# AlexTate/ShortSeq

Measured on AMD Instinct MI355X. Metric: nt/sec 2-bit encode (32/96/512-nt batches) + hamming pairs/sec; % HBM roofline, higher is better.
Workload: dtype u8; 1 GPU; C2: 100M x 32-nt batch encode (short_seq_64 path) per GPU; reads_per_gpu=100000000, read_len=32, global_batch=100000000, parallelism=dp1 (read shards, no collective)

## Files before the change

### shortseq_amd/csrc/ss_counter.hip

```cpp
#include "ss_device.h"
#include "ss_internal.h"

using namespace ssd;

namespace {
struct alignas(16) Slot {
    unsigned long long key;
    uint32_t ncount;
    uint32_t first;
};
static_assert(sizeof(Slot) == 16, "one slot = one dwordx4");
constexpr uint32_t kNoFirst = 0xFFFFFFFFu;
constexpr uint64_t kMaxIndex = 0xFFFFFFFEull;
constexpr unsigned long long kOvfTable = 1ull, kOvfExtract = 2ull, kOvfField = 4ull, kOvfIndex = 8ull;
constexpr int kThreads = 256;
constexpr uint32_t kMaxParts = 64;
constexpr uint32_t kExtractBlocks = 4096;
constexpr uint32_t kExtractT = 64;
constexpr uint32_t kSliceLogMax = 11;
constexpr uint32_t kMwSliceLog = 11;
constexpr uint32_t kPartBlocks = 1024;
constexpr uint32_t kMaxRegions = 32768;
}

// ... 1156 lines not shown
        const bool heavy_tile = any_heavy != 0;
#pragma unroll
        for (int j = 0; j < (int)(kTile / T); ++j) {
            const uint32_t e = j * T + threadIdx.x;
            if (e < cnt) {
                const uint32_t sp = lstart[lb[j]] + rank[j];
                skey[sp] = key[j];
                sidx[sp] = idx[j];
            }
        }
        if (heavy_tile)
            for (uint32_t i = threadIdx.x; i < kTile; i += T) ht[i] = 0;
        __syncthreads();
        if (heavy_tile) {
            for (uint32_t i0 = 0; i0 < cnt; i0 += T) {
                const uint32_t i = i0 + threadIdx.x;
                const uint64_t k = i < cnt ? skey[i] : 0ull;
                const uint32_t x = i < cnt ? sidx[i] : kWeighted;
                const bool act = i < cnt && lcount[region_of_h(t, k) - r0] > heavy_at && !(x & kWeighted);
                if (!act) continue;
                uint32_t h = dedup_home(k, kHtLog);
                for (;;) {
                    uint32_t e = ht[h];
                    if (e == 0) {
                        e = atomicCAS(&ht[h], 0u, (i + 1) | (1u << 16));
                        if (e == 0) break;
                    }
                    const uint32_t j = (e & 0xFFFFu) - 1;
                    if (skey[j] == k) {
                        atomicAdd(&ht[h], 1u << 16);
                        atomicMin(&sidx[j], x);
                        sidx[i] = kDead;
                        break;
                    }
                    h = (h + 1) & (kTile - 1);
                }
            }
            __syncthreads();
            for (uint32_t i = threadIdx.x; i < cnt; i += T) {
                const uint32_t b = region_of_h(t, skey[i]) - r0;
                if (lcount[b] > heavy_at && sidx[i] != kDead) atomicAdd(&hcnt[b], 1u);
            }
            for (uint32_t i = threadIdx.x; i < nb; i += T)
                if (lcount[i] > heavy_at) lstart[i] = 0;
            __syncthreads();
        }
#pragma unroll
        for (int j = 0; j < (int)(kTile / T); ++j) asm volatile("" ::"v"(nkey[j]), "v"(nidx[j]));
        for (uint32_t i = threadIdx.x; i < cnt; i += T) {
            const uint64_t k = skey[i];
            const uint32_t x = sidx[i];
            if (x == kDead) continue;
            const uint32_t b = region_of_h(t, k) - r0;
            uint32_t local, c = 1;
            if (heavy_tile && lcount[b] > heavy_at) {
                local = atomicAdd(&lstart[b], 1u);
                if (!(x & kWeighted)) {
                    uint32_t h = dedup_home(k, kHtLog);
                    while ((ht[h] & 0xFFFFu) != i + 1) h = (h + 1) & (kTile - 1);
                    c = ht[h] >> 16;
                }
            } else {
                local = i - lstart[b];
            }
            uint32_t xi = x;
            if (x & kWeighted) {
                const uint32_t p = x & ~kWeighted;
                xi = srec[p].idx;
                c = src_cnt[p];
            } else if (c > 1) {
                xi = x | kWeighted;
            }
            const uint32_t gpos = cursor[b] + local;
            if (w.slab && gpos >= sbase + (b + 1) * ssize) {
                const uint64_t sp = atomicAdd(w.spill_ctr, 1u);
                const uint64_t key = k * kSlotInv;
                if (sp < w.spill_cap)
                    w.spill[sp] = make_uint4((uint32_t)key, (uint32_t)(key >> 32), c, xi & ~kWeighted);
                else
                    atomicOr(t.overflow, kOvfTable);
                continue;
            }
            if (c > 1) w.bcnt[gpos] = c;
            Rec12 r;
            r.klo = (uint32_t)k;
            r.khi = (uint32_t)(k >> 32);
            r.idx = xi;
            ((Rec12*)w.keys)[gpos] = r;
        }
        __syncthreads();
        for (uint32_t i = threadIdx.x; i < nb; i += T)
            cursor[i] += (heavy_tile && lcount[i] > heavy_at) ? hcnt[i] : lcount[i];
        __syncthreads();
    }
    for (uint32_t i = threadIdx.x; i < nb; i += T)
        w.seg_end[(uint64_t)fb * nb + i] = w.slab ? min(cursor[i], sbase + (i + 1) * ssize) : cursor[i];
}

__global__ __launch_bounds__(256) void k_spill_insert(Tbl t, PartWs w, const uint32_t* __restrict__ fill,
                                                      uint64_t base_index) {
    const uint64_t m = min((uint64_t)fill[fill_at(kSpillCtr)], w.spill_cap);
    for (uint64_t i0 = (uint64_t)blockIdx.x * 256; i0 < m; i0 += (uint64_t)gridDim.x * 256) {
        const uint64_t i = i0 + threadIdx.x;
        const uint4 r = w.spill[min(i, m - 1)];
        const uint64_t k = ((uint64_t)r.y << 32) | r.x;
        bool act = i < m;
        uint32_t c = r.z, idx = r.w;
        wave_fold<kSpillFold, true>(act, k, c, idx);
        if (act && tbl_add(t, k, c, base_index + idx) && t.occ && k != kEmpty) atomicAdd(&t.occ[region_of(t, k)], 1u);
    }
}


constexpr uint32_t kAggSliceT = 512;
constexpr int kAggP = 4;


constexpr int kAggProbe = 2;
constexpr int kAggProbeS = 4;
template <int G>
__device__ __forceinline__ bool lds_probe_round(unsigned long long* skey, uint32_t mask, uint64_t empty, uint64_t k,
                                                uint32_t& off, uint32_t& done, uint32_t& at) {
    const uint32_t S = mask + 1;
    unsigned long long cur[G];
#pragma unroll
    for (int g = 0; g < G; ++g) cur[g] = skey[(off + g) & mask];
    int hit = -1;
    bool free_at = false;
#pragma unroll
    for (int g = G - 1; g >= 0; --g) {
        if (cur[g] == k) {
            hit = g;
            free_at = false;
        } else if (cur[g] == empty) {
            hit = g;
            free_at = true;
        }
    }
    if (hit >= 0) {
        at = (off + (uint32_t)hit) & mask;
        if (!free_at) return true;
        const unsigned long long prev = atomicCAS(&skey[at], (unsigned long long)empty, (unsigned long long)k);
        if (prev == empty || prev == k) return true;
        off = (at + 1) & mask;
        done += (uint32_t)hit + 1;
    } else {
        off = (off + G) & mask;
        done += G;
    }
    at = S;
    return done >= S;
}

template <int T, bool REC12>
__global__ __launch_bounds__(T) void k_pc_aggregate_slice(Tbl t, PartWs w, uint64_t base_index, bool fresh = false) {
    const uint32_t S = (uint32_t)t.slice_mask + 1;
    extern __shared__ __attribute__((aligned(16))) unsigned char smem[];
    unsigned long long* skey = (unsigned long long*)smem;
    uint32_t* bcnt = (uint32_t*)(skey + S);
    uint32_t* bfst = bcnt + S;
    __shared__ uint32_t sent[3];
    const uint32_t region = blockIdx.x;
    const uint64_t slice_base = (uint64_t)region << t.slice_log;
    static_assert(kFinePerBin <= 32, "segment table: two lanes per segment");
    const uint32_t lane = threadIdx.x & 63u;
    uint32_t meta;
    if (w.seg_end) {
        const uint32_t rpb = 1u << (w.rbits - kCoarseBits);
        const uint32_t sg = lane % kFinePerBin;
        const uint64_t at = (uint64_t)((region / rpb) * kFinePerBin + sg) * rpb + region % rpb;
        meta = (lane < kFinePerBin ? w.hist : w.seg_end)[at];
    } else {
        meta = w.rstart[region + (lane & 1u)];
    }
    constexpr uint64_t kE = REC12 ? kEmptyH : kEmpty;
    if (fresh) {
        for (uint32_t i = threadIdx.x; i < S; i += T) skey[i] = kE;
    } else {
        for (uint32_t i = threadIdx.x; i < S; i += T) {
            const uint64_t k = t.slots[slice_base + i].key;
            skey[i] = REC12 ? (k == kEmpty ? kEmptyH : k * kSlotMul) : k;
        }
    }
    for (uint32_t i = threadIdx.x; i < S; i += T) {
        bcnt[i] = 0;
        bfst[i] = 0xFFFFFFFFu;
    }
    if (threadIdx.x == 0) {
        sent[0] = 0;
        sent[1] = 0xFFFFFFFFu;
        sent[2] = 0;
    }
    constexpr int kP = kAggP;
    uint32_t seg0[kFinePerBin], pre[kFinePerBin + 1];
    pre[0] = 0;
    if (w.seg_end) {
#pragma unroll
        for (uint32_t sg = 0; sg < kFinePerBin; ++sg) {
            seg0[sg] = (uint32_t)__builtin_amdgcn_readlane((int)meta, (int)sg);
            pre[sg + 1] = pre[sg] + ((uint32_t)__builtin_amdgcn_readlane((int)meta, (int)(kFinePerBin + sg)) - seg0[sg]);
        }
    } else {
        seg0[0] = (uint32_t)__builtin_amdgcn_readlane((int)meta, 0);
        const uint32_t end = (uint32_t)__builtin_amdgcn_readlane((int)meta, 1);
#pragma unroll
        for (uint32_t sg = 0; sg < kFinePerBin; ++sg) pre[sg + 1] = end - seg0[0];
    }
    const uint32_t total = pre[kFinePerBin];
    auto flat_at = [&](uint32_t f) -> uint32_t {
        uint32_t e = seg0[0] + f;
#pragma unroll
        for (uint32_t sg = 1; sg < kFinePerBin; ++sg)
            if (f >= pre[sg]) e = seg0[sg] + (f - pre[sg]);
        return e;
    };
    uint64_t nkey[kP];
    uint32_t nidx[kP], nel[kP];
    auto load_step = [&](uint32_t e0) {
#pragma unroll
        for (int q = 0; q < kP; ++q) {
            const uint32_t f = min(e0 + q * T + threadIdx.x, total - 1u);
            nel[q] = flat_at(f);
            if constexpr (REC12) {
                const Rec12 r = w.brec[nel[q]];
                nkey[q] = ((uint64_t)r.khi << 32) | r.klo;
                nidx[q] = r.idx;
            } else {
                nkey[q] = w.bkey[nel[q]];
                nidx[q] = w.bidx[nel[q]];
            }
        }
    };
    if (total) load_step(0);
    auto home_of = [&](uint64_t k) -> uint64_t {
        return REC12 ? (t.shift >= 64 ? 0ull : k >> t.shift) : slot_top(t, k);
    };
    auto probe_round = [&](uint64_t k, uint32_t& off, uint32_t& done, uint32_t& at) -> bool {
        return lds_probe_round<kAggProbe>(skey, (uint32_t)t.slice_mask, kE, k, off, done, at);
    };
    auto probe_round_s = [&](uint64_t k, uint32_t& off, uint32_t& done, uint32_t& at) -> bool {
        return lds_probe_round<kAggProbeS>(skey, (uint32_t)t.slice_mask, kE, k, off, done, at);
    };
    auto commit = [&](uint32_t at, uint32_t c, uint32_t ix) {
        if (at == S) {
            atomicOr(t.overflow, kOvfTable);
        } else {
            atomicAdd(&bcnt[at], c);
            atomicMin(&bfst[at], ix);
        }
    };
    __syncthreads();
    for (uint32_t e0 = 0; e0 < total; e0 += kP * T) {
        uint64_t key[kP];
        uint32_t idx[kP], el[kP];
#pragma unroll
        for (int q = 0; q < kP; ++q) {
            key[q] = nkey[q];
            idx[q] = nidx[q];
            el[q] = nel[q];
        }
        uint32_t cw[kP];
#pragma unroll
        for (int q = 0; q < kP; ++q) {
            const bool valid = e0 + q * T + threadIdx.x < total;
            cw[q] = (valid && (idx[q] & kWeighted)) ? w.bcnt[el[q]] : 1u;
        }
        load_step(e0 + kP * T);
        uint32_t pend = 0, soff[kP];
#pragma unroll
        for (int q = 0; q < kP; ++q) {
            const bool valid = e0 + q * T + threadIdx.x < total;
            soff[q] = 0;
            if (valid && key[q] == kE) {
                atomicAdd(&sent[0], cw[q]);
                atomicMin(&sent[1], idx[q] & ~kWeighted);
            }
            if (!valid || key[q] == kE) continue;
            uint32_t off = (uint32_t)(home_of(key[q]) & t.slice_mask), done = 0, at;
            if (probe_round(key[q], off, done, at))
                commit(at, cw[q], idx[q] & ~kWeighted);
            else {
                pend |= 1u << q;
                soff[q] = off;
            }
        }
        if (__ballot(pend != 0)) {
            uint64_t k = 0;
            uint32_t off = 0, done = 0, c = 0, ix = 0;
            auto pick = [&]() {
#pragma unroll
                for (int q = kP - 1; q >= 0; --q)
                    if (pend & (1u << q)) {
                        k = key[q];
                        off = soff[q];
                        c = cw[q];
                        ix = idx[q] & ~kWeighted;
                    }
                done = (off - (uint32_t)home_of(k)) & (uint32_t)t.slice_mask;
            };
            if (pend) pick();
            while (__ballot(pend != 0)) {
                uint32_t at;
                if (pend && probe_round_s(k, off, done, at)) {
                    commit(at, c, ix);
                    pend &= pend - 1u;
                    if (pend) pick();
                }
            }
        }
    }
    __syncthreads();
    uint32_t used = 0;
    uint4* sl = (uint4*)&t.slots[slice_base];
    for (uint32_t i = threadIdx.x; i < S; i += T) {
        const unsigned long long kh = skey[i];
        used += kh != kE ? 1u : 0u;
        const unsigned long long k = REC12 ? (kh != kE ? kh * kSlotInv : kEmpty) : kh;
        const uint32_t bc = bcnt[i];
        if (fresh) {
            sl[i] = make_uint4((uint32_t)k, (uint32_t)(k >> 32), ~bc,
                               bc ? (uint32_t)(base_index + bfst[i]) : kNoFirst);
        } else if (bc) {
            const uint4 old = sl[i];
            const uint32_t f = (uint32_t)(base_index + bfst[i]);
            sl[i] = make_uint4((uint32_t)k, (uint32_t)(k >> 32), old.z - bc, f < old.w ? f : old.w);
        }
    }
    if (t.occ) {
        if (used) atomicAdd(&sent[2], used);
        __syncthreads();
        if (threadIdx.x == 0) t.occ[region] = sent[2];
    }
    if (threadIdx.x == 0 && sent[0]) {
        Slot* ss = &t.slots[t.mask + 1];
        atomicAdd(&ss->ncount, 0u - sent[0]);
        atomicMin(&ss->first, (uint32_t)(base_index + sent[1]));
    }
}

struct TripleRecs {
    const uint64_t* keys;
    const uint64_t* counts;
    const uint64_t* first;
    __device__ __forceinline__ uint64_t key(uint64_t j) const { return keys[j]; }
    __device__ __forceinline__ void load(uint64_t j, uint32_t, uint64_t& k, unsigned long long& c,
                                         unsigned long long& f) const {
        k = keys[j];
        c = counts[j];
        f = first[j];
    }
};

struct PackedRecs {
    const uint4* rec;
    const uint64_t* run_base;
    __device__ __forceinline__ uint64_t key(uint64_t j) const {
        const uint4 v = rec[j];
        return ((uint64_t)v.y << 32) | v.x;
    }
    __device__ __forceinline__ void load(uint64_t j, uint32_t run, uint64_t& k, unsigned long long& c,
                                         unsigned long long& f) const {
        const uint4 v = rec[j];
        k = ((uint64_t)v.y << 32) | v.x;
        c = v.z;
        f = run_base[run] + v.w;
    }
};

template <typename Recs>
__device__ __forceinline__ uint32_t run_rel(const Tbl& t, const Recs& recs, uint64_t j, uint32_t reg_lo, uint32_t nreg) {
    const uint64_t k = recs.key(j);
    if (k == kEmpty) return nreg;
    const uint32_t r = region_of(t, k);
    return r < reg_lo ? 0u : min(r - reg_lo, nreg);
}

template <typename Recs>
__global__ __launch_bounds__(256) void k_run_bounds(Tbl t, Recs recs,
                                                   const uint64_t* __restrict__ run_off, uint32_t n_runs,
                                                   uint32_t reg_lo, uint32_t nreg, uint32_t* __restrict__ bounds) {
    const uint64_t i = (uint64_t)blockIdx.x * 256 + threadIdx.x;
    uint32_t run = 0;
    while (run < n_runs && !(run_off[2 * run] <= i && i < run_off[2 * run + 1])) ++run;
    if (run == n_runs) return;
    const uint64_t beg = run_off[2 * run], end = run_off[2 * run + 1];
    auto rel = [&](uint64_t j) { return run_rel(t, recs, j, reg_lo, nreg); };
    const uint32_t r = rel(i);
    const uint32_t prev = i == beg ? 0u : rel(i - 1) + 1u;
    uint32_t* b = bounds + (uint64_t)run * (nreg + 1);
    for (uint32_t q = (i == beg ? 0u : prev); q <= r; ++q) b[q] = (uint32_t)(i - beg);
    if (i + 1 == end)
        for (uint32_t q = r + 1; q <= nreg; ++q) b[q] = (uint32_t)(end - beg);
}

constexpr uint32_t kMergeT = 512;
constexpr uint32_t kMergeSearchRuns = 64;
constexpr int kMergeK = 4;

template <typename Recs>
__global__ __launch_bounds__(kMergeT) void k_merge_runs(Tbl t, Recs recs,
                                                       const uint64_t* __restrict__ run_off, uint32_t n_runs,
                                                       uint32_t reg_lo, uint32_t nreg,
                                                       const uint32_t* __restrict__ bounds) {
    extern __shared__ __attribute__((aligned(16))) unsigned char smem[];
    const uint32_t S = (uint32_t)t.slice_mask + 1;
    unsigned long long* skey = (unsigned long long*)smem;
    uint32_t* scnt = (uint32_t*)(skey + S);
    uint32_t* sfst = scnt + S;
    const uint32_t j = blockIdx.x;
    const uint64_t base = (uint64_t)(reg_lo + j) << t.slice_log;
    uint4* sl = (uint4*)&t.slots[base];
    for (uint32_t q = threadIdx.x; q < S; q += kMergeT) {
        const uint4 v = sl[q];
        skey[q] = ((uint64_t)v.y << 32) | v.x;
        scnt[q] = ~v.z;
        sfst[q] = v.w;
    }
    __shared__ uint32_t s_lo[kMergeSearchRuns], s_hi[kMergeSearchRuns];
    if (!bounds) {
        const uint32_t hl = threadIdx.x & 31u, hsh = threadIdx.x & 32u;
        for (uint32_t q = threadIdx.x >> 5; q < 2 * n_runs; q += kMergeT / 32) {
            const uint32_t run = q >> 1, target = j + (q & 1u);
            const uint64_t beg = run_off[2 * run], end = run_off[2 * run + 1];
            uint64_t L = beg, H = end;
            while (H > L) {
                const uint64_t len = H - L;
                const uint64_t p = L + len * hl / 32;
                const bool below = run_rel(t, recs, p, reg_lo, nreg) < target;
                const uint32_t c = (uint32_t)__popcll((__ballot(below) >> hsh) & 0xFFFFFFFFull);
                if (c == 0) break;
                const uint64_t nx = c < 32 ? L + len * c / 32 : H;
                L = L + len * (c - 1) / 32 + 1;
                H = nx;
            }
            if (hl == 0) ((q & 1u) ? s_hi : s_lo)[run] = (uint32_t)(L - beg);
        }
    }
// ... 1414 lines not shown
    c->ws_bidx = nullptr;
    c->ws_bcnt = nullptr;
    c->ws_spill = nullptr;
    c->ws_reads = 0;
    c->ws_slab = 0;
    c->ws_brecs = 0;
    return SS_OK;
}

static int insert_impl(ss_counter* c, const uint8_t* d_ascii, uint64_t n, uint32_t L, uint64_t stride,
                       uint64_t base_index, uint64_t* d_first_bad, void* stream, const uint64_t* words_in,
                       const uint64_t* keys_in = nullptr) {
    hipStream_t s = (hipStream_t)stream;
    int rc = SS_OK;
    if (keys_in) {
        if (c->W != 1) return ss_fail(SS_EARG, "precomputed keys need a single-word handle");
        if (n == 0) return SS_OK;
        if (n > c->ws_reads && (rc = ss_counter_reserve(c, n)) != SS_OK) return rc;
    }
    const uint32_t rb = c->log2cap - c->slice_log;
    const bool opt = !words_in && n > 0 && n <= c->ws_reads && rb > kCoarseBits && rb - kCoarseBits <= 8 &&
                     (keys_in || (d_ascii && (L == 16 || L == 32) && stride % 16 == 0 && (((uintptr_t)d_ascii) & 15) == 0));
    if (keys_in) {
    } else if (!words_in) {
        if (!d_first_bad) return ss_fail(SS_EARG, "d_first_bad is required");
        if (stride < L) return ss_fail(SS_EARG, "stride < L");
        if ((rc = fix_length(c, L))) return rc;
        if (!opt) rc = ss_check(set_u64(d_first_bad, true, s), "reset first_bad");
        if (rc || n == 0) return rc;
        if (!d_ascii) return ss_fail(SS_EARG, "null buffer");
    } else if (n == 0) {
        return SS_OK;
    }
    if (base_index > kMaxIndex || n - 1 > kMaxIndex - base_index)
        return ss_fail(SS_EARG, "global read indices of a counter handle must stay below 2^32 - 1");
    if (c->L != kWordKeys && c->since + n > c->spill_at && (rc = spill_wide(c, s))) return rc;
    c->since += n;
    c->occ_src = 0;
    Tbl t = tbl_of(c);
    const bool multi = c->W > 1;
    const bool fast = !words_in && !keys_in && (L == 16 || L == 32) && stride % 16 == 0 && (((uintptr_t)d_ascii) & 15) == 0;
    const uint64_t* mw = words_in;
    if (multi) {
        if (n > c->ws_reads && (rc = ss_counter_reserve(c, n)) != SS_OK) return rc;
    }
    if (multi && !words_in) {
        const uint64_t need = c->ws_reads * c->W;
        if (c->ws_words_cap < need) {
            if (c->ws_words) (void)hipFree(c->ws_words);
            c->ws_words = nullptr;
            c->ws_words_cap = 0;
            if (hipMalloc((void**)&c->ws_words, need * sizeof(uint64_t)) != hipSuccess) {
                ss_check(hipGetLastError(), "counter word workspace hipMalloc");
                return ss_fail(SS_ENOMEM, "counter word workspace: out of device memory");
            }
            c->ws_words_cap = need;
        }
        rc = ss_encode_fixed_impl(d_ascii, n, L, stride, c->ws_words, c->W, d_first_bad, nullptr, nullptr, stream);
        if (rc) return rc;
        mw = c->ws_words;
    }
    const bool packed_keys = !multi && !fast && n <= c->ws_reads;
    if (packed_keys && keys_in && !opt) {
        rc = ss_check(hipMemcpyAsync(c->ws_keys, keys_in, n * 8, hipMemcpyDeviceToDevice, s), "counter key copy");
        if (rc) return rc;
    } else if (packed_keys && !keys_in) {
        rc = ss_encode_fixed_impl(d_ascii, n, L, stride, c->ws_keys, 1, d_first_bad, nullptr, nullptr, stream);
        if (rc) return rc;
    }
    const bool part = multi || packed_keys || (fast && n <= c->ws_reads);
    bool fresh = false;
    if (part && !multi) {
        fresh = c->reset_pending;
        c->reset_pending = false;
    } else if ((rc = flush_reset(c, s)) != SS_OK) {
        return rc;
    }
    if (part) {
        PartWs w;
        w.keys = c->ws_keys;
        w.akey = c->ws_akey;
        w.aidx = c->ws_aidx;
        w.acnt = c->ws_acnt;
        w.areg = c->ws_areg;
        w.bidx = c->ws_bidx;
        w.bcnt = c->ws_bcnt;
        w.spill = c->ws_spill;
        w.spill_cap = c->ws_reads;
        w.seg_end = nullptr;
        w.hist = c->ws_hist;
        w.rstart = c->ws_rstart;
        w.tot = c->ws_tot;
        w.bkey = nullptr;
        w.brec = nullptr;
        w.slab = 0;
        w.slabs = nullptr;
        w.spill_ctr = nullptr;
        w.R = (uint32_t)(c->cap >> c->slice_log);
        w.rbits = c->log2cap - c->slice_log;
        const uint32_t S = 1u << c->slice_log;
        const size_t mw_lds = (size_t)2 * S * 16 + (size_t)S * 8;
        const bool two_pass = w.rbits > kCoarseBits;
        const uint32_t bins1 = two_pass ? (1u << kCoarseBits) : w.R;
        constexpr int T1 = 512, U1 = 2, TS = 512, TF = 512;
        static const hipError_t attrs = [] {
            const int agg_max = (int)(2 * (1u << kMwSliceLog) * 16 + (1u << kMwSliceLog) * 8 + 8);
            hipError_t ea = hipFuncSetAttribute((const void*)k_pc_keys<T1, U1>,
                                                hipFuncAttributeMaxDynamicSharedMemorySize, kMaxRegions * 4);
            if (ea == hipSuccess)
                ea = hipFuncSetAttribute((const void*)k_pc_hist<TF>, hipFuncAttributeMaxDynamicSharedMemorySize,
                                         kMaxRegions * 4);
            for (int f = 0; f < kMwAggFns && ea == hipSuccess; ++f)
                ea = hipFuncSetAttribute((const void*)kMwFp[f], hipFuncAttributeMaxDynamicSharedMemorySize,
                                         kMaxRegions * 4);
            for (int f = 0; f < kMwAggFns && ea == hipSuccess; ++f)
                ea = hipFuncSetAttribute((const void*)kMwAgg[f], hipFuncAttributeMaxDynamicSharedMemorySize, agg_max);

            return ea;
        }();
        if (attrs != hipSuccess) return ss_check(attrs, "hipFuncSetAttribute (dynamic LDS)");
        auto scan = [&](uint32_t bins, uint32_t* start) {
            hipLaunchKernelGGL(k_pc_tot, dim3(bins), dim3(256), 0, s, w, bins);
            hipLaunchKernelGGL(k_pc_scan, dim3(1), dim3(1024), 0, s, w, bins, start);
            hipLaunchKernelGGL(k_pc_offsets, dim3(bins), dim3(1024), 0, s, w, bins, (const uint32_t*)start);
        };
        if (!multi && (!packed_keys || (keys_in && opt)) && two_pass && w.rbits - kCoarseBits <= 8) {
            const uint64_t cap1 = c->ws_cap1;
            w.slab = (uint32_t)c->ws_slab;
            w.spill_ctr = c->ws_fill + fill_at(kSpillCtr);
            hipEvent_t tev[ss_counter::kPassEvents] = {};
            for (uint32_t p = 0; p < ss_counter::kPassEvents; ++p) tev[p] = timer_event(c, p);
            auto mark = [&](uint32_t p) {
                if (tev[p]) (void)hipEventRecord(tev[p], s);
            };
            mark(0);
            PrepWords pw{};
            pw.p[0] = (unsigned long long*)d_first_bad;
            pw.v[0] = ~0ull;
            pw.zero = c->ws_fill;
            pw.nzero = kFillWords;
            rc = ss_check(launch_prep(pw, s), "first_bad / fill reset");
            if (rc) return rc;
            static const int pf_grid = [] {
                int dev = 0, cus = 0, per = 0;
                (void)hipGetDevice(&dev);
                (void)hipDeviceGetAttribute(&cus, hipDeviceAttributeMultiprocessorCount, dev);
                (void)hipOccupancyMaxActiveBlocksPerMultiprocessor(&per, (const void*)k_pf_coarse<kPfT, kPfRPL, false, true>, kPfT, 0);
                return (cus > 0 && per > 0) ? cus * per : (int)kPartBlocks;
            }();
            if (keys_in)
                hipLaunchKernelGGL((k_pf_coarse<kPfT, kPfRPL, true, false>), dim3(pf_grid), dim3(kPfT), 0, s, t, w,
                                   (const uint4*)keys_in, (uint64_t)0, n, 0u, cap1, c->ws_fill,
                                   (unsigned long long*)nullptr);
            else if (L == 32)
                hipLaunchKernelGGL((k_pf_coarse<kPfT, kPfRPL, false, true>), dim3(pf_grid), dim3(kPfT), 0, s, t, w,
                                   (const uint4*)d_ascii, stride / 16, n, 2u, cap1, c->ws_fill,
                                   (unsigned long long*)d_first_bad);
            else
                hipLaunchKernelGGL((k_pf_coarse<kPfT, kPfRPL, false, false>), dim3(pf_grid), dim3(kPfT), 0, s, t, w,
                                   (const uint4*)d_ascii, stride / 16, n, L / 16, cap1, c->ws_fill,
                                   (unsigned long long*)d_first_bad);
            const unsigned fine_blocks = kCB * kFinePerBin;
            if (!w.slab) {
                hipLaunchKernelGGL((k_pf_count<512>), dim3(fine_blocks), dim3(512), 0, s, t, w, cap1,
                                   (const uint32_t*)c->ws_fill);
                const unsigned rg = (w.R + 255) / 256;
                hipLaunchKernelGGL(k_pf_tot, dim3(rg), dim3(256), 0, s, w);
                hipLaunchKernelGGL(k_pc_scan, dim3(1), dim3(1024), 0, s, w, w.R, w.rstart, (const uint32_t*)nullptr);
                hipLaunchKernelGGL(k_pf_offsets, dim3(rg), dim3(256), 0, s, w);
            }
            w.seg_end = c->ws_segend;
            w.slabs = w.slab ? c->ws_order + kNFill : nullptr;
            mark(1);
            hipLaunchKernelGGL(k_pf_order, dim3(1), dim3(512), 0, s, (const uint32_t*)c->ws_fill, cap1, c->ws_order,
                               1u << (w.rbits - kCoarseBits), w.slab ? c->ws_order + kNFill : nullptr);
            mark(2);
            hipLaunchKernelGGL((k_pf_scatter<kFsT, kFsTile>), dim3(fine_blocks), dim3(kFsT), 0, s, t, w, cap1,
                               (const uint32_t*)c->ws_fill, (const uint32_t*)c->ws_order);
            mark(3);
            w.bkey = w.keys;
            w.brec = (const Rec12*)w.keys;
            hipLaunchKernelGGL((k_pc_aggregate_slice<kAggSliceT, true>), dim3(w.R), dim3(kAggSliceT),
                               ((size_t)1 << c->slice_log) * 16, s, t, w, base_index, fresh);
            mark(4);
            hipLaunchKernelGGL(k_spill_insert, dim3(1024), dim3(256), 0, s, t, w, (const uint32_t*)c->ws_fill,
                               base_index);
            mark(5);
            if (c->tev) {
                c->thead = (c->thead + 1) % ss_counter::kTimerRing;
                ++c->tpend;
            }
            c->occ_src = 1;
            return ss_check(hipGetLastError(), "optimistic partitioned insert");
        }
        if (multi) {
            const size_t fp_lds = (bins1 * (TF / 64) <= kMaxRegions ? bins1 * (TF / 64) : bins1) * 4;
            static_assert(TF == kMwFpT, "k_mw_fp instances");
            hipLaunchKernelGGL(kMwFp[mw_variant(t.W, mw)], dim3(kPartBlocks), dim3(TF), fp_lds, s, t, w, bins1, mw, n);
        } else if (packed_keys) {
            const size_t h_lds = (bins1 * (TF / 64) <= kMaxRegions ? bins1 * (TF / 64) : bins1) * 4;
            hipLaunchKernelGGL((k_pc_hist<TF>), dim3(kPartBlocks), dim3(TF), h_lds, s, t, w, bins1, n);
        } else {
            const size_t keys_lds = (bins1 * (T1 / 64) <= kMaxRegions ? bins1 * (T1 / 64) : bins1) * 4;
            hipLaunchKernelGGL((k_pc_keys<T1, U1>), dim3(kPartBlocks), dim3(T1), keys_lds, s, t, w, bins1,
                               (const uint4*)d_ascii, stride / 16, n, L / 16, (unsigned long long*)d_first_bad);
        }
        if (two_pass) {
            scan(bins1, w.tot + 0);
            hipLaunchKernelGGL((k_pc_scatter_lds<true, false>), dim3(kPartBlocks), dim3(512), 0, s, t, w, bins1,
                               (const uint64_t*)w.keys, (const uint32_t*)nullptr, w.akey, w.aidx, n);
            hipLaunchKernelGGL((k_pc_count<TS>), dim3(kPartBlocks), dim3(TS), 0, s, t, w, (const uint64_t*)w.akey, n);
            scan(w.R, w.rstart);
            hipLaunchKernelGGL((k_pc_scatter_lds<false, true>), dim3(kPartBlocks), dim3(512), 0, s, t, w, w.R,
                               (const uint64_t*)w.akey, (const uint32_t*)w.aidx, w.keys, w.bidx, n);
            w.bkey = w.keys;
        } else {
            scan(w.R, w.rstart);
            hipLaunchKernelGGL((k_pc_scatter_lds<true, false>), dim3(kPartBlocks), dim3(512), 0, s, t, w, w.R,
                               (const uint64_t*)w.keys, (const uint32_t*)nullptr, w.akey, w.bidx, n);
            w.bkey = w.akey;
        }
        if (multi)
            hipLaunchKernelGGL(kMwAgg[mw_variant(t.W, mw)], dim3(w.R), dim3(kMwT), mw_lds, s, t, w, mw, base_index);
        else
            hipLaunchKernelGGL((k_pc_aggregate_slice<kAggSliceT, false>), dim3(w.R), dim3(kAggSliceT),
                               ((size_t)1 << c->slice_log) * 16, s, t, w, base_index, fresh);
        if (!multi) c->occ_src = 1;
        return ss_check(hipGetLastError(), "partitioned insert");
    }
    if (fast) {
        constexpr int U = 4;
        const unsigned grid = grid_for(2 * n, (uint64_t)U * kThreads, 0);
        hipLaunchKernelGGL((k_count_g16<U>), dim3(grid), dim3(kThreads), 0, s, t, (const uint4*)d_ascii,
                           stride / 16, n, L / 16, base_index, (unsigned long long*)d_first_bad);
        return ss_check(hipGetLastError(), "k_count_g16");
    }
    const unsigned grid = grid_for(n, kThreads, 256 * 16);
    hipLaunchKernelGGL(k_count_gen, dim3(grid), dim3(kThreads), 0, s, t, d_ascii, stride, n, L, base_index,
                       (unsigned long long*)d_first_bad);
    return ss_check(hipGetLastError(), "k_count_gen");
}

int ss_counter_insert_fixed(ss_counter* c, const uint8_t* d_ascii, uint64_t n, uint32_t L,
                            uint64_t stride, uint64_t base_index, uint64_t* d_first_bad, void* stream) {
    if (!c) return ss_fail(SS_EARG, "null counter");
    if (c->L == kWordKeys) return ss_fail(SS_EARG, "the handle holds packed multi-word keys (ss_counter_insert_words)");
    return insert_impl(c, d_ascii, n, L, stride, base_index, d_first_bad, stream, nullptr);
}

int ss_counter_set_words(ss_counter* c, uint32_t W) {
    if (!c) return ss_fail(SS_EARG, "null counter");
    if (W < 2 || W > 64) return ss_fail(SS_EARG, "packed keys of 2..64 words");
    if (c->L == kWordKeys && c->W == W) return SS_OK;
    if (c->L != -1) return ss_fail(SS_EARG, "the handle already holds keys of another kind");
    if (c->keywords_W != W) {
        if (c->keywords) (void)hipFree(c->keywords);
        c->keywords = nullptr;
        c->keywords_W = 0;
        if (hipMalloc((void**)&c->keywords, c->cap * W * sizeof(uint64_t)) != hipSuccess) {
            ss_check(hipGetLastError(), "counter key words hipMalloc");
            return ss_fail(SS_ENOMEM, "counter key words: out of device memory");
        }
        c->keywords_W = W;
    }
    c->W = W;
    c->L = kWordKeys;
    return SS_OK;
}

int ss_counter_insert_words(ss_counter* c, const uint64_t* d_words, uint64_t n, uint64_t base_index, void* stream) {
    if (!c) return ss_fail(SS_EARG, "null counter");
    if (c->L != kWordKeys) return ss_fail(SS_EARG, "ss_counter_set_words first");
    if (n && !d_words) return ss_fail(SS_EARG, "null buffer");
    return insert_impl(c, nullptr, n, 0, 0, base_index, nullptr, stream, d_words);
}

int ss_counter_insert_keys(ss_counter* c, const uint64_t* d_keys, uint64_t n, uint64_t base_index, void* stream) {
    if (!c) return ss_fail(SS_EARG, "null counter");
    if (n && !d_keys) return ss_fail(SS_EARG, "null buffer");
    if (c->L < 0) {
        const int rc = fix_length(c, 32);
        if (rc) return rc;
    }
    return insert_impl(c, nullptr, n, 0, 0, base_index, nullptr, stream, nullptr, d_keys);
}

int ss_counter_merge(ss_counter* c, const uint64_t* d_keys, const uint32_t* d_lens,
                     const uint64_t* d_counts, const uint64_t* d_first, uint64_t m, void* stream) {
    (void)d_lens;
    if (!c) return ss_fail(SS_EARG, "null counter");
    if (m == 0) return SS_OK;
    if (!d_keys || !d_counts || !d_first) return ss_fail(SS_EARG, "null buffer");
    if (c->W > 1) return ss_fail(SS_EARG, "ss_counter_merge takes single-word keys (L <= 32)");
    const unsigned grid = grid_for(m, kThreads, 256 * 16);
    c->occ_src = 0;
    int rc = flush_reset(c, (hipStream_t)stream);
    if (!rc) rc = wide_on(c, (hipStream_t)stream);
    if (rc) return rc;
    c->since = kSinceUnknown;
    hipLaunchKernelGGL(k_merge, dim3(grid), dim3(kThreads), 0, (hipStream_t)stream, tbl_of(c), d_keys, d_counts,
                       d_first, m);
    return ss_check(hipGetLastError(), "k_merge");
}

int ss_counter_merge_words(ss_counter* c, const uint64_t* d_words, const uint64_t* d_counts,
                           const uint64_t* d_first, uint64_t m, void* stream) {
    if (!c) return ss_fail(SS_EARG, "null counter");
// ... 345 lines not shown
```

Measured before the change: 5293 billion nt/s.

## Assign one wave per fine segment and use branchless first LDS probe in aggregation

In the REC12 aggregate-slice kernel, each wave now walks its own fine segment directly instead of every thread mapping a flat index through a prefix table, which removes the per-element segment search. The first hash probe becomes a branchless gather-then-CAS helper, and weighted-count loads and sentinel atomics now run only when some lane in the wave needs them. The L==32 coarse-path selection also gains a 32-bit offset guard. Walking per wave can leave waves unevenly loaded when segment sizes differ, and it relies on the block size matching the segment count.

```diff
diff --git a/shortseq_amd/csrc/ss_counter.hip b/shortseq_amd/csrc/ss_counter.hip
--- a/shortseq_amd/csrc/ss_counter.hip
+++ b/shortseq_amd/csrc/ss_counter.hip
@@ -1332,6 +1332,32 @@
     return done >= S;
 }
 
+template <int G>
+__device__ __forceinline__ bool lds_probe_first(unsigned long long* skey, uint32_t mask, uint64_t empty, uint64_t k,
+                                                bool act, uint32_t home, uint32_t& off, uint32_t& done, uint32_t& at) {
+    unsigned long long cur[G];
+#pragma unroll
+    for (int g = 0; g < G; ++g) cur[g] = skey[(home + g) & mask];
+    uint32_t hit = G;
+    bool is_free = false;
+#pragma unroll
+    for (int g = G - 1; g >= 0; --g) {
+        const bool m = cur[g] == k, e = cur[g] == empty;
+        hit = (m | e) ? (uint32_t)g : hit;
+        is_free = (m | e) ? (e & !m) : is_free;
+    }
+    at = (home + hit) & mask;
+    bool fin = act & (hit < G) & !is_free, lost = false;
+    if (act & (hit < G) & is_free) {
+        const unsigned long long prev = atomicCAS(&skey[at], (unsigned long long)empty, (unsigned long long)k);
+        fin = (prev == empty) | (prev == k);
+        lost = !fin;
+    }
+    off = lost ? (at + 1) & mask : (home + G) & mask;
+    done = lost ? hit + 1 : (uint32_t)G;
+    return fin;
+}
+
 template <int T, bool REC12>
 __global__ __launch_bounds__(T) void k_pc_aggregate_slice(Tbl t, PartWs w, uint64_t base_index, bool fresh = false) {
     const uint32_t S = (uint32_t)t.slice_mask + 1;
@@ -1345,7 +1371,7 @@
     static_assert(kFinePerBin <= 32, "segment table: two lanes per segment");
     const uint32_t lane = threadIdx.x & 63u;
     uint32_t meta;
-    if (w.seg_end) {
+    if constexpr (REC12) {
         const uint32_t rpb = 1u << (w.rbits - kCoarseBits);
         const uint32_t sg = lane % kFinePerBin;
         const uint64_t at = (uint64_t)((region / rpb) * kFinePerBin + sg) * rpb + region % rpb;
@@ -1372,51 +1398,37 @@
         sent[2] = 0;
     }
     constexpr int kP = kAggP;
-    uint32_t seg0[kFinePerBin], pre[kFinePerBin + 1];
-    pre[0] = 0;
-    if (w.seg_end) {
-#pragma unroll
-        for (uint32_t sg = 0; sg < kFinePerBin; ++sg) {
-            seg0[sg] = (uint32_t)__builtin_amdgcn_readlane((int)meta, (int)sg);
-            pre[sg + 1] = pre[sg] + ((uint32_t)__builtin_amdgcn_readlane((int)meta, (int)(kFinePerBin + sg)) - seg0[sg]);
-        }
+    constexpr uint32_t kWalk = REC12 ? 64u : (uint32_t)T;
+    const uint32_t wl = REC12 ? lane : threadIdx.x;
+    uint32_t seg0, total;
+    if constexpr (REC12) {
+        static_assert(T / 64 == (int)kFinePerBin, "one wave per fine segment");
+        const int wv = __builtin_amdgcn_readfirstlane((int)(threadIdx.x >> 6));
+        seg0 = (uint32_t)__builtin_amdgcn_readlane((int)meta, wv);
+        total = (uint32_t)__builtin_amdgcn_readlane((int)meta, (int)kFinePerBin + wv) - seg0;
     } else {
-        seg0[0] = (uint32_t)__builtin_amdgcn_readlane((int)meta, 0);
-        const uint32_t end = (uint32_t)__builtin_amdgcn_readlane((int)meta, 1);
-#pragma unroll
-        for (uint32_t sg = 0; sg < kFinePerBin; ++sg) pre[sg + 1] = end - seg0[0];
-    }
-    const uint32_t total = pre[kFinePerBin];
-    auto flat_at = [&](uint32_t f) -> uint32_t {
-        uint32_t e = seg0[0] + f;
-#pragma unroll
-        for (uint32_t sg = 1; sg < kFinePerBin; ++sg)
-            if (f >= pre[sg]) e = seg0[sg] + (f - pre[sg]);
-        return e;
-    };
+        seg0 = (uint32_t)__builtin_amdgcn_readlane((int)meta, 0);
+        total = (uint32_t)__builtin_amdgcn_readlane((int)meta, 1) - seg0;
+    }
     uint64_t nkey[kP];
-    uint32_t nidx[kP], nel[kP];
+    uint32_t nidx[kP];
     auto load_step = [&](uint32_t e0) {
 #pragma unroll
         for (int q = 0; q < kP; ++q) {
-            const uint32_t f = min(e0 + q * T + threadIdx.x, total - 1u);
-            nel[q] = flat_at(f);
+            const uint32_t e = seg0 + min(e0 + q * kWalk + wl, total - 1u);
             if constexpr (REC12) {
-                const Rec12 r = w.brec[nel[q]];
+                const Rec12 r = w.brec[e];
                 nkey[q] = ((uint64_t)r.khi << 32) | r.klo;
                 nidx[q] = r.idx;
             } else {
-                nkey[q] = w.bkey[nel[q]];
-                nidx[q] = w.bidx[nel[q]];
+                nkey[q] = w.bkey[e];
+                nidx[q] = w.bidx[e];
             }
         }
     };
     if (total) load_step(0);
     auto home_of = [&](uint64_t k) -> uint64_t {
         return REC12 ? (t.shift >= 64 ? 0ull : k >> t.shift) : slot_top(t, k);
-    };
-    auto probe_round = [&](uint64_t k, uint32_t& off, uint32_t& done, uint32_t& at) -> bool {
-        return lds_probe_round<kAggProbe>(skey, (uint32_t)t.slice_mask, kE, k, off, done, at);
     };
     auto probe_round_s = [&](uint64_t k, uint32_t& off, uint32_t& done, uint32_t& at) -> bool {
         return lds_probe_round<kAggProbeS>(skey, (uint32_t)t.slice_mask, kE, k, off, done, at);
@@ -1430,39 +1442,57 @@
         }
     };
     __syncthreads();
-    for (uint32_t e0 = 0; e0 < total; e0 += kP * T) {
+    for (uint32_t e0 = 0; e0 < total; e0 += kP * kWalk) {
         uint64_t key[kP];
-        uint32_t idx[kP], el[kP];
+        uint32_t idx[kP];
 #pragma unroll
         for (int q = 0; q < kP; ++q) {
             key[q] = nkey[q];
             idx[q] = nidx[q];
-            el[q] = nel[q];
         }
         uint32_t cw[kP];
+        bool valid[kP], wtd = false;
 #pragma unroll
         for (int q = 0; q < kP; ++q) {
-            const bool valid = e0 + q * T + threadIdx.x < total;
-            cw[q] = (valid && (idx[q] & kWeighted)) ? w.bcnt[el[q]] : 1u;
-        }
-        load_step(e0 + kP * T);
+            valid[q] = e0 + q * kWalk + wl < total;
+            cw[q] = 1u;
+            wtd |= valid[q] & ((idx[q] & kWeighted) != 0u);
+        }
+        if (__ballot(wtd)) {
+#pragma unroll
+            for (int q = 0; q < kP; ++q)
+                if (valid[q] && (idx[q] & kWeighted)) cw[q] = w.bcnt[seg0 + e0 + q * kWalk + wl];
+        }
+        load_step(e0 + kP * kWalk);
         uint32_t pend = 0, soff[kP];
+        bool sen = false;
+#pragma unroll
+        for (int q = 0; q < kP; ++q) sen |= valid[q] & (key[q] == kE);
+        if (__ballot(sen)) {
+#pragma unroll
+            for (int q = 0; q < kP; ++q)
+                if (valid[q] && key[q] == kE) {
+                    atomicAdd(&sent[0], cw[q]);
+                    atomicMin(&sent[1], idx[q] & ~kWeighted);
+                }
+        }
 #pragma unroll
         for (int q = 0; q < kP; ++q) {
-            const bool valid = e0 + q * T + threadIdx.x < total;
-            soff[q] = 0;
-            if (valid && key[q] == kE) {
-                atomicAdd(&sent[0], cw[q]);
-                atomicMin(&sent[1], idx[q] & ~kWeighted);
-            }
-            if (!valid || key[q] == kE) continue;
-            uint32_t off = (uint32_t)(home_of(key[q]) & t.slice_mask), done = 0, at;
-            if (probe_round(key[q], off, done, at))
-                commit(at, cw[q], idx[q] & ~kWeighted);
-            else {
-                pend |= 1u << q;
-                soff[q] = off;
-            }
+            const bool act = valid[q] & (key[q] != kE);
+            uint32_t off, done, at;
+            const bool fin = lds_probe_first<kAggProbe>(skey, (uint32_t)t.slice_mask, kE, key[q], act,
+                                                        (uint32_t)(home_of(key[q]) & t.slice_mask), off, done, at);
+            if (fin) {
+                atomicAdd(&bcnt[at], cw[q]);
+                atomicMin(&bfst[at], idx[q] & ~kWeighted);
+            }
+            bool more = act & !fin;
+            if (S <= (uint32_t)kAggProbe) {
+                if (more && done >= S) commit(S, 0u, 0u);
+                more &= done < S;
+            }
+            pend |= more ? 1u << q : 0u;
+            soff[q] = more ? off : 0u;
         }
         if (__ballot(pend != 0)) {
             uint64_t k = 0;
@@ -3183,7 +3213,7 @@
                 hipLaunchKernelGGL((k_pf_coarse<kPfT, kPfRPL, true, false>), dim3(pf_grid), dim3(kPfT), 0, s, t, w,
                                    (const uint4*)keys_in, (uint64_t)0, n, 0u, cap1, c->ws_fill,
                                    (unsigned long long*)nullptr);
-            else if (L == 32)
+            else if (L == 32 && (uint64_t)(kPfT * kPfRPL) * (stride / 16) < (1ull << 32))
                 hipLaunchKernelGGL((k_pf_coarse<kPfT, kPfRPL, false, true>), dim3(pf_grid), dim3(kPfT), 0, s, t, w,
                                    (const uint4*)d_ascii, stride / 16, n, 2u, cap1, c->ws_fill,
                                    (unsigned long long*)d_first_bad);
```

Result: no change. 5294 billion nt/s (median of 4 runs) (+0.0%).
